# liuQuan98/APR

Hardware: AMD Instinct MI355X
Metric: point-cloud pairs/sec (120k-pt KITTI frame, FCGF encode+match+SVD) (higher is better)
Workload: dtype f32

## Files before the change

apr_amd/_lib.py:

```python
from __future__ import annotations

import ctypes as C
import os

import torch

_HERE = os.path.dirname(os.path.abspath(__file__))
LIB_PATH = os.path.join(_HERE, "lib", "libapr_hip.so")

_p = C.c_void_p
_i32, _i64, _u64, _f32, _f64, _sz = C.c_int32, C.c_int64, C.c_uint64, C.c_float, C.c_double, C.c_size_t

class PairDesc(C.Structure):
    _fields_ = [("f0", C.c_void_p), ("n0", C.c_int64), ("f1", C.c_void_p), ("n1", C.c_int64),
                ("xyz0", C.c_void_p), ("xyz1", C.c_void_p), ("seed", C.c_uint64)]


class SpconvDesc(C.Structure):
    _fields_ = [("inp", C.c_void_p), ("ldi", C.c_int64), ("nbr", C.c_void_p), ("n_out", C.c_int64),
                ("K", C.c_int32), ("cin", C.c_int32), ("cout", C.c_int32), ("relu", C.c_int32),
                ("w_packed", C.c_void_p), ("scale", C.c_void_p), ("shift", C.c_void_p),
                ("residual", C.c_void_p), ("ldr", C.c_int64), ("out", C.c_void_p), ("ldo", C.c_int64),
                ("counters", C.c_void_p), ("plist", C.c_void_p), ("prod_scratch", C.c_void_p),
                ("plist_bytes", C.c_int64), ("w_bf3", C.c_void_p),
# ... 21 lines not shown
    _fields_ = [("layer", ResunetLayer * 23), ("conv1_w", C.c_void_p), ("conv1_ks", C.c_int32), ("normalize", C.c_int32),
                ("ws_conv", C.c_uint32), ("ws_block", C.c_uint32), ("os_block", C.c_uint32),
                ("ws3", C.c_int32), ("ws3_cin128", C.c_int32), ("os_min_rows", C.c_int32), ("occ_kernel_map", C.c_int32),
                ("ws3_max_rows_128", C.c_int64)]


class LevelMap(C.Structure):
    _fields_ = [("coords", C.c_void_p), ("keys", C.c_void_p), ("vals", C.c_void_p), ("cap", C.c_int64), ("n", C.c_int64)]


class Pyramid(C.Structure):
    _fields_ = [("lv", LevelMap * 4), ("first", C.c_void_p), ("pts", C.c_void_p), ("header", C.c_void_p),
                ("header_ints", C.c_int32), ("compact", C.c_int32), ("compact_rows", C.c_int64),
                ("counters", C.c_void_p), ("n_counter_slots", C.c_int32)]


class GcnLayer(C.Structure):
    _fields_ = [("kind", C.c_int32), ("k", C.c_int32), ("heads", C.c_int32),
                ("eps1", C.c_float), ("eps2", C.c_float), ("eps3", C.c_float),
                ("w1", C.c_void_p), ("w2", C.c_void_p), ("w3", C.c_void_p), ("b1", C.c_void_p), ("b2", C.c_void_p),
                ("wq", C.c_void_p), ("wk", C.c_void_p), ("wv", C.c_void_p), ("wm", C.c_void_p),
                ("bq", C.c_void_p), ("bk", C.c_void_p), ("bv", C.c_void_p), ("bm", C.c_void_p)]


class GcnDesc(C.Structure):
    _fields_ = [("n_layers", C.c_int32), ("c", C.c_int32), ("layer", GcnLayer * 8)]


PROTOTYPES = {
    "apr_col_sums": (C.c_int, [_p, _i64, _i64, _i32, _p, _p, _sz, _p]),
    "apr_mha_train_forward": (C.c_int, [_p, _p, _p, _i32, _i32, _i32, _i32, _i32, _p, _p, _p]),
    "apr_mha_train_backward": (C.c_int, [_p, _p, _p, _p, _p, _i32, _i32, _i32, _i32, _i32, _p, _p, _p, _p, _p]),
    "apr_edge_features_backward": (C.c_int, [_p, _i32, _i32, _i32, _p, _i64, _p, _p]),
    "apr_gcn_scratch_bytes": (_sz, [_p, _i32, _i32]),
    "apr_gcn_forward": (C.c_int, [_p, _p, _i32, _p, _i32, _p, _i64, _p, _i64, _p, _i64, _p, _i64, _p, _sz, _p]),
    "apr_voxel_pyramid_scratch_bytes": (_sz, [_i64, _i32]),
    "apr_voxel_pyramid": (C.c_int, [_p, _p, _i32, _f32, _p, _sz, _p, _p]),
    "apr_resunet_encode_supported": (C.c_int, [_p, _p, _p]),
    "apr_resunet_encode_scratch_bytes": (_sz, [_p, _p, _p]),
    "apr_resunet_encode": (C.c_int, [_p, _p, _p, _p, _i32, _p, _sz, _p, _i64, _p]),
    "apr_last_error": (C.c_char_p, []),
    "apr_version": (C.c_int, []),
    "apr_device_count": (C.c_int, []),
    "apr_struct_sizes": (_i32, [_p, _i32]),
    "apr_ransac_set_screen": (C.c_int, [_i32]),
    "apr_ransac_set_option": (C.c_int, [_i32, _i32]),
    "apr_ransac_sampling_launches": (C.c_int, [_p]),
    "apr_event_wait": (C.c_int, [_p, _i32]),
    "apr_event_wait_timeout": (C.c_int, [_p, _i32, _i64]),
    "apr_hash_capacity": (_i64, [_i64]),
    "apr_map_scratch_bytes": (_sz, [_i64]),
    "apr_voxelize": (C.c_int, [_p, _i64, _f32, _i32, _p, _p]),
    "apr_map_build": (C.c_int, [_p, _i64, _p, _i32, _p, _p, _i64, _p, _p, _p, _p, _p, _sz, _p]),
    "apr_kernel_map_transpose": (C.c_int, [_p, _i64, _i32, _i64, _p, _p]),
    "apr_voxelize_segments": (C.c_int, [_p, _i64, C.c_float, _p, _i32, _p, _p]),
    "apr_segment_counts": (C.c_int, [_p, _p, _p, _i32, _p, _p]),
    "apr_kernel_map_same": (C.c_int, [_p, _i64, _p, _p, _i64, _i32, _i32, _p, _p]),
    "apr_kernel_map": (C.c_int, [_p, _i64, _p, _p, _p, _i64, _i32, _i32, _p, _p]),
    "apr_spconv_packed_size": (_i64, [_i32, _i32, _i32]),
    "apr_spconv_pack_weights": (C.c_int, [_p, _i32, _i32, _i32, _p, _p]),
    "apr_spconv_fwd": (C.c_int, [_p, _i64, _p, _i64, _i32, _i32, _i32, _p, _p, _p, _p, _i64, _i32, _p, _i64, _p]),
    "apr_pairlist_counter_ints": (_i32, []),
    "apr_pairlist_bytes": (_sz, [_i64, _i32]),
    "apr_pairlist_build": (C.c_int, [_p, _i64, _i32, _p, _p, _sz, _p]),
    "apr_pairlist3_bytes": (_sz, [_i64]),
    "apr_pairlist3_build": (C.c_int, [_p, _i64, _i32, _p, _p, _sz, _p]),
    "apr_spconv_ws3_supported": (C.c_int, [_i32, _i32, _i32]),
    "apr_spconv_ws3_fwd_bf3": (C.c_int, [_p, _i64, _p, _p, _i64, _i32, _i32, _p, _p, _p, _p, _i64, _i32, _p, _i64, _p, _p]),
    "apr_spconv_ws_fwd": (C.c_int, [_p, _i64, _p, _p, _i64, _i32, _i32, _i32, _p, _p, _p, _p, _i64, _i32, _p, _i64, _p, _p]),
    "apr_spconv_packed_bf3_bytes": (_i64, [_i32, _i32, _i32]),
    "apr_spconv_pack_weights_bf3": (C.c_int, [_p, _i32, _i32, _i32, _p, _p]),
    "apr_spconv_pack_weights_bf3_ex": (C.c_int, [_p, _i32, _i32, _i32, _i32, _i32, _p, _p]),
    "apr_spconv_ws_fwd_bf3": (C.c_int, [_p, _i64, _p, _p, _i64, _i32, _i32, _i32, _p, _p, _p, _p, _p, _i64, _i32, _p, _i64,
                                        _p, _p]),
    "apr_spconv_wgrad_scratch_bytes": (_sz, [_i64, _i32, _i32, _i32]),
    "apr_spconv_wgrad": (C.c_int, [_p, _i64, _p, _i64, _p, _i64, _i32, _i32, _i32, _p, _p, _sz, _p]),
    "apr_spconv_wgrad_same_level": (C.c_int, [_p, _i64, _p, _i64, _p, _i64, _i32, _i32, _i32, _p, _p, _sz, _p]),
    "apr_spconv_route": (_i32, [_p]),
    "apr_spconv_tile_variant": (_i32, [_p]),
    "apr_dense_gemm_bf3_variant": (_i32, [_i64, _i32, _i32]),
    "apr_spconv_wgrad_plan": (C.c_int, [_p, _i64, _p, _i64, _i64, _i32, _i32, _i32, _i32, _p]),
    "apr_spconv_ws_supported": (_i32, [_i32, _i32, _i32]),
    "apr_spconv_bigk_supported": (_i32, [_i32, _i32, _i32]),
    "apr_spconv_fwd_batch": (C.c_int, [_p, _i32, _p]),
    "apr_spconv_fwd_batch_timed": (C.c_int, [_p, _i32, _p, _p]),
    "apr_bn_stats": (C.c_int, [_p, _i64, _i64, _i32, _p, _p, _p, _sz, _p]),
    "apr_norm_params": (C.c_int, [_p, _i64, _i64, _i32, _f32, _p, _p, _p, _sz, _p]),
    "apr_bn_stats_scratch_bytes": (_sz, [_i64, _i32]),
    "apr_instance_norm_act": (C.c_int, [_p, _i64, _i64, _i32, _f32, _p, _i64, _i32, _f32, _p, _i64, _p, _sz, _p]),
    "apr_spconv_os_tile_rows": (_i32, [_i64, _i32, _i32]),
    "apr_spconv_os_pairs_bytes": (_sz, [_i64, _i32, _i32]),
    "apr_spconv_os_pairs_build": (C.c_int, [_p, _i64, _i64, _i32, _i32, _p, _sz, _p]),
    "apr_spconv_os_trace": (C.c_int, [_p, _i32]),
    "apr_spconv_os_set_debug": (C.c_int, [_i32]),
    "apr_spconv_os_fwd": (C.c_int, [_p, _i64, _p, _i64, _i32, _i32, _i32, _i32, _p, _p, _p, _p, _i64, _i32, _p, _i64, _p]),
    "apr_norm_backward_scratch_bytes": (_sz, [_i64, _i32]),
    "apr_norm_backward": (C.c_int, [_p, _i64, _p, _i64, _i64, _i32, _p, _p, _p, _p, _i64, _p, _p, _p, _sz, _p]),
    "apr_bn_train_fwd": (C.c_int, [_p, _i64, _i64, _i32, _p, _p, C.c_float, C.c_float, _p, _p, _p, _i64, _i32, _p, _i64, _p, _p,
                                   _p, _p, _i32, _p, _sz, _p]),
    "apr_bn_train_bwd": (C.c_int, [_p, _i64, _p, _i64, _p, _i64, _i64, _i32, _p, _p, _p, _i32, _p, _i64, _p, _i64, _p, _p,
                                   _p, _i32, _p, _sz, _p]),
    "apr_weights_flip_transpose": (C.c_int, [_p, _i32, _i32, _i32, _i32, _p, _p]),
    "apr_dense_gemm_bf3": (C.c_int, [_p, _i64, _i64, _i32, _i32, _p, _p, _p, _p, _i64, _i32, _p, _i64, _p]),
    "apr_dense_rows_bf3_ok": (_i32, [_i32, _i32]),
    "apr_dense_rows_bf3_route": (_i32, [_i64, _i32, _i32]),
    "apr_dense_rows_bf3": (C.c_int, [_p, _i64, _i64, _i32, _i32, _p, _p, _p, _p, _i64, _i32, _i32, _p, _i64, _p]),
# ... 195 lines not shown
```

apr_amd/csrc/encoder.hip:

```cpp
#include "common.h"

namespace {

constexpr int kLevels = 4, kStages = 7, kMaps = 10, kMaxLists = 24;

struct ListSlot {
  int map, kind, rows;
  void* blob;
  size_t bytes;
  int32_t* counters;
  bool built;
};

struct Enc {
  const apr_resunet_plan& P;
  const apr_level_map* lv;
  const int32_t* bbox;
  AprArena arena;
  const bool dry;
  hipStream_t st;
  int rc = APR_OK;

  int32_t* kmap[kMaps] = {};
  ListSlot lists[kMaxLists];
  int nlists = 0, ncounter = 0;
  int32_t* counters = nullptr;
  int n_counter_slots = 0;
  void* occ = nullptr;
  size_t occ_bytes = 0;
  int32_t* tpool[3] = {};
  bool tpool_ready = false;
  float* prod = nullptr;
  size_t prod_bytes = 0;

  apr_spconv_desc descs[4];
  int ndesc = 0;

  Enc(const apr_resunet_plan& p, const apr_level_map* l, const int32_t* b, void* scratch, hipStream_t s)
      : P(p), lv(l), bbox(b), arena(scratch), dry(scratch == nullptr), st(s) {}

  float* rows(int64_t n, int c) { return arena.take<float>((size_t)n * c); }
  size_t need() const { return arena.bytes() + apr_align256(prod_bytes); }
  bool ok() const { return rc == APR_OK; }
  void run(int r) {
    if (rc == APR_OK && r != APR_OK) rc = r;
  }

  int64_t map_rows(int m) const { return m < 4 ? lv[m].n : m < 7 ? lv[m - 4 + 1].n : lv[m - 7].n; }
  int64_t map_in_rows(int m) const { return m < 4 ? lv[m].n : m < 7 ? lv[m - 4].n : lv[m - 7 + 1].n; }

  int32_t* kernel_map(int m) {
    if (kmap[m] || (dry && kmap_sized[m])) return kmap[m];
    kmap_sized[m] = true;
    const int64_t n_out = map_rows(m);
    if (m >= 7) {
      const int l = m - 7;
      int32_t* fwd = kernel_map(4 + l);
      if (!tpool_ready) {
        size_t ints = 0;
        for (int a = 0; a < 3; ++a) ints += (size_t)lv[a].n * 27;
        ints = (ints + 63) / 64 * 64 + 64;
        int32_t* buf = arena.take<int32_t>(ints);
        size_t pos = 0;
        for (int a = 0; a < 3; ++a) {
          tpool[a] = dry ? nullptr : buf + pos;
          pos += (size_t)lv[a].n * 27;
        }
        if (!dry) run(apr_fill_bytes(buf, 0xFF, ints * 4, st));
        tpool_ready = true;
      }
      kmap[m] = tpool[l];
      if (!dry) run(apr_kernel_map_transpose_prefilled(fwd, lv[l + 1].n, 27, lv[l].n, kmap[m], st));
      return kmap[m];
    }
    kmap[m] = arena.take<int32_t>((size_t)n_out * 27);
    if (dry) return kmap[m];
    const int lin = m < 4 ? m : m - 4, lout = m < 4 ? m : m - 4 + 1;
    const apr_level_map& in = lv[lin];
    const apr_level_map& outm = lv[lout];
    if (lin == 0 && P.occ_kernel_map && occ)
      run(apr_kernel_map_occ(outm.coords, outm.n, nullptr, in.keys, in.vals, in.cap, 3, 1, bbox, P.conv1_ks, occ, kmap[m], st));
    else
      run(apr_kernel_map(outm.coords, outm.n, nullptr, in.keys, in.vals, in.cap, 3, 1 << lin, kmap[m], st));
    return kmap[m];
  }
  bool kmap_sized[kMaps] = {};

  ListSlot* find_list(int m, int kind, int rws) {
    for (int i = 0; i < nlists; ++i)
      if (lists[i].map == m && lists[i].kind == kind && lists[i].rows == rws) return &lists[i];
    return nullptr;
  }

  ListSlot* ws_list(const apr_resunet_layer& L, int m, bool same_level) {
    bool tri = P.ws3 && L.w_bf3 && apr_spconv_ws3_supported(L.K, L.cin, L.cout);
    if (tri && L.cin == 128 && ((same_level && map_rows(m) > P.ws3_max_rows_128) || !P.ws3_cin128)) tri = false;
    const int kind = tri ? 1 : 0;
    ListSlot* s = find_list(m, kind, 0);
    if (s) return s;
    if (nlists >= kMaxLists) {
      apr_set_error("apr_resunet_encode: more than %d pair lists", kMaxLists);
      run(APR_EINVAL);
      return nullptr;
    }
    s = &lists[nlists++];
    s->map = m;
    s->kind = kind;
    s->rows = 0;
    s->bytes = tri ? apr_pairlist3_bytes(map_rows(m)) : apr_pairlist_bytes(map_rows(m), 27);
    s->blob = arena.take<char>(s->bytes);
    s->built = false;
    s->counters = nullptr;
    if (!dry) {
      if (ncounter >= n_counter_slots) {
        apr_set_error("apr_resunet_encode: more than %d pair lists need a counter block", n_counter_slots);
        run(APR_EINVAL);
        return nullptr;
      }
      s->counters = counters + (size_t)ncounter * apr_pairlist_counter_ints();
    }
    ++ncounter;
    return s;
  }

  ListSlot* os_list(const apr_resunet_layer& L, int m) {
    const int64_t n_out = map_rows(m), n_in = map_in_rows(m);
    const int rws = n_in < (1ll << 23) ? apr_spconv_os_tile_rows(n_out, L.cin, L.cout) : 0;
    if (rws <= 0) return nullptr;
    ListSlot* s = find_list(m, 2, rws);
    if (s) return s;
    if (nlists >= kMaxLists) {
      apr_set_error("apr_resunet_encode: more than %d pair lists", kMaxLists);
      run(APR_EINVAL);
      return nullptr;
    }
    s = &lists[nlists++];
// ... 130 lines not shown
  const apr_resunet_layer* L = p->layer;
  for (int s = 0; s < kStages; ++s)
    if (L[3 * s + 1].cin != L[3 * s].cout || L[3 * s + 1].cout != L[3 * s].cout || L[3 * s + 2].cin != L[3 * s].cout ||
        L[3 * s + 2].cout != L[3 * s].cout)
      return false;
  if (L[3].cin != L[0].cout || L[6].cin != L[3].cout || L[9].cin != L[6].cout || L[12].cin != L[9].cout ||
      L[15].cin != L[12].cout + L[6].cout || L[18].cin != L[15].cout + L[3].cout || L[21].cin != L[18].cout + L[0].cout ||
      L[22].cin != L[21].cout)
    return false;
  if (L[0].cin != 1 || L[0].K != p->conv1_ks * p->conv1_ks * p->conv1_ks || L[0].cout % 8 != 0) return false;
  if (p->conv1_ks != 3 && p->conv1_ks != 5 && p->conv1_ks != 7) return false;
  return true;
}

}

APR_API int apr_resunet_encode_supported(const apr_resunet_plan* plan, const apr_level_map* lv, const int32_t* bbox_host) {
  if (!plan_ok(plan, lv, bbox_host)) return 0;
  return apr_occ_conv_pays(bbox_host, plan->conv1_ks, lv[0].n) ? 1 : 0;
}

APR_API size_t apr_resunet_encode_scratch_bytes(const apr_resunet_plan* plan, const apr_level_map* lv, const int32_t* bbox_host) {
  if (!apr_resunet_encode_supported(plan, lv, bbox_host)) return 0;
  Enc e(*plan, lv, bbox_host, nullptr, nullptr);
  e.walk(nullptr, plan->layer[22].cout);
  return e.need();
}

APR_API int apr_resunet_encode(const apr_resunet_plan* plan, const apr_level_map* lv, const int32_t* bbox_host, int32_t* counters,
                               int32_t n_counter_slots, void* scratch, size_t scratch_bytes, float* out, int64_t ldo,
                               void* stream) {
  APR_CHECK_ARG(apr_resunet_encode_supported(plan, lv, bbox_host),
                "apr_resunet_encode: plan / maps / box not covered (apr_resunet_encode_supported)");
  APR_CHECK_ARG(scratch && out && ldo >= plan->layer[22].cout && (!counters || n_counter_slots > 0),
                "apr_resunet_encode: bad arguments");
  Enc dry(*plan, lv, bbox_host, nullptr, nullptr);
  dry.walk(nullptr, ldo);
  APR_CHECK_ARG(scratch_bytes >= dry.need(), "apr_resunet_encode: scratch too small");
  Enc e(*plan, lv, bbox_host, scratch, (hipStream_t)stream);
  e.counters = counters;
  e.n_counter_slots = counters ? n_counter_slots : 0;
  e.prod_bytes_live = dry.prod_bytes;
  e.walk(out, ldo);
  return e.rc;
}

namespace {

struct MapBufs {
  uint64_t* keys; int32_t* vals; int64_t cap; int32_t* coords; int64_t* first; int32_t *n_dev, *status; void* scratch;
  size_t scratch_bytes; int64_t rows;
};

MapBufs take_map(AprArena& f, int64_t rows, bool want_first, int32_t* hdr_slot, void* shared_scratch, size_t shared_bytes) {
  MapBufs m;
  m.rows = rows;
  m.cap = apr_hash_capacity(rows);
  m.keys = f.take<uint64_t>((size_t)m.cap);
  m.vals = f.take<int32_t>((size_t)m.cap);
  m.coords = f.take<int32_t>((size_t)rows * 4);
  m.first = want_first ? f.take<int64_t>((size_t)rows) : nullptr;
  m.scratch_bytes = shared_bytes;
  m.scratch = shared_scratch;
  m.n_dev = hdr_slot;
  m.status = hdr_slot ? hdr_slot + 1 : nullptr;
  return m;
}

inline int64_t compact_rows_for(int64_t n_points) { return n_points > 4 * 65536 ? (n_points / 4 > 65536 ? n_points / 4 : 65536) : 0; }

int front_walk(AprArena& f, const float* const* frames, const int64_t* offs, int32_t nseg, float vs, apr_pyramid* out,
               hipStream_t st) {
  const int64_t N = offs ? offs[nseg] : 0;
  const int64_t R = compact_rows_for(N);
  const int hints = 10 + nseg + 8;
  const bool dry = f.base == nullptr;
  int32_t* hdr = f.take<int32_t>((size_t)hints);
  int32_t* counters = f.take<int32_t>((size_t)16 * apr_pairlist_counter_ints());
  int32_t* raw = f.take<int32_t>((size_t)N * 4);
  int64_t* offs_dev = f.take<int64_t>((size_t)(nseg + 1));
  float* pts = f.take<float>((size_t)N * 3);
  const size_t sbytes = apr_map_scratch_bytes(N);
  void* const sc = f.take<char>(sbytes);
  MapBufs dedup = take_map(f, N, true, dry ? nullptr : hdr + (R ? 8 : 0), sc, sbytes);
  MapBufs lvl[4];
  if (R) lvl[0] = take_map(f, R, false, dry ? nullptr : hdr, sc, sbytes);
  else lvl[0] = dedup;
  const int64_t rows = R ? R : N;
  for (int l = 1; l < 4; ++l) lvl[l] = take_map(f, rows, false, dry ? nullptr : hdr + 2 * l, sc, sbytes);
  if (dry) return APR_OK;

  int rc;
  const size_t clear = (size_t)((char*)counters - (char*)hdr) + (size_t)16 * apr_pairlist_counter_ints() * 4;
  if ((rc = apr_pack_i32(nullptr, nullptr, 0, nullptr, hdr, (int64_t)(clear / 4), st)) != APR_OK) return rc;
  if ((rc = apr_voxelize_frames(frames, offs, nseg, vs, raw, offs_dev, st)) != APR_OK) return rc;
  if ((rc = apr_map_build(raw, N, nullptr, 0, dedup.keys, dedup.vals, dedup.cap, dedup.coords, dedup.first, dedup.n_dev,
                          dedup.status, dedup.scratch, dedup.scratch_bytes, st)) != APR_OK)
    return rc;
  if ((rc = apr_segment_counts(dedup.first, dedup.n_dev, offs_dev, nseg, hdr + 10, st)) != APR_OK) return rc;
  if ((rc = apr_coords_bbox(raw, N, hdr + 10 + nseg, st)) != APR_OK) return rc;
  if ((rc = apr_gather_frame_points(frames, offs, nseg, dedup.first, dedup.n_dev, N, pts, st)) != APR_OK) return rc;
  if (R &&
      (rc = apr_map_build(dedup.coords, R, dedup.n_dev, 0, lvl[0].keys, lvl[0].vals, lvl[0].cap, lvl[0].coords, nullptr,
                          lvl[0].n_dev, lvl[0].status, lvl[0].scratch, lvl[0].scratch_bytes, st)) != APR_OK)
    return rc;
  for (int l = 1; l < 4; ++l)
    if ((rc = apr_map_build(lvl[l - 1].coords, rows, lvl[l - 1].n_dev, 1 << l, lvl[l].keys, lvl[l].vals, lvl[l].cap, lvl[l].coords,
                            nullptr, lvl[l].n_dev, lvl[l].status, lvl[l].scratch, lvl[l].scratch_bytes, st)) != APR_OK)
      return rc;
  for (int l = 0; l < 4; ++l) {
    out->lv[l].coords = lvl[l].coords; out->lv[l].keys = lvl[l].keys; out->lv[l].vals = lvl[l].vals;
    out->lv[l].cap = lvl[l].cap; out->lv[l].n = lvl[l].rows;
  }
  out->first = dedup.first;
  out->pts = pts;
  out->header = hdr;
  out->header_ints = hints;
  out->compact = R ? 1 : 0;
  out->compact_rows = R;
  out->counters = counters;
  out->n_counter_slots = 16;
  return APR_OK;
}

}

APR_API size_t apr_voxel_pyramid_scratch_bytes(int64_t n_points, int32_t nseg) {
  if (n_points <= 0 || nseg <= 0 || nseg > APR_MAX_FRAMES) return 0;
  AprArena f(nullptr);
  int64_t offs[APR_MAX_FRAMES + 1] = {};
  offs[nseg] = n_points;
  (void)front_walk(f, nullptr, offs, nseg, 1.f, nullptr, nullptr);
  return f.bytes();
}

APR_API int apr_voxel_pyramid(const float* const* frames_host, const int64_t* offsets_host, int32_t nseg, float voxel_size,
                              void* arena, size_t arena_bytes, apr_pyramid* out, void* stream) {
  APR_CHECK_ARG(frames_host && offsets_host && nseg >= 1 && nseg <= APR_MAX_FRAMES && arena && out && voxel_size > 0.f,
                "apr_voxel_pyramid: bad arguments (1 .. %d frames)", APR_MAX_FRAMES);
  APR_CHECK_ARG(offsets_host[0] == 0 && offsets_host[nseg] > 0, "apr_voxel_pyramid: offsets must run 0 .. total points > 0");
  APR_CHECK_ARG(arena_bytes >= apr_voxel_pyramid_scratch_bytes(offsets_host[nseg], nseg), "apr_voxel_pyramid: arena too small");
  AprArena f(arena);
  return front_walk(f, frames_host, offsets_host, nseg, voxel_size, out, (hipStream_t)stream);
}
```

apr_amd/csrc/hash.hip:

```cpp
#include "common.h"

namespace {

constexpr int kBlock = 256;

__global__ void k_voxelize(const float* __restrict__ xyz, int64_t n, float vs, int batch,
                           int4* __restrict__ coords) {
  int64_t i = (int64_t)blockIdx.x * blockDim.x + threadIdx.x;
  if (i >= n) return;
  float x = xyz[3 * i + 0] / vs, y = xyz[3 * i + 1] / vs, z = xyz[3 * i + 2] / vs;
  coords[i] = make_int4(batch, (int)floorf(x), (int)floorf(y), (int)floorf(z));
}

__global__ void k_voxelize_segments(const float* __restrict__ xyz, int64_t n, float vs,
                                    const long long* __restrict__ offsets, int nseg, int4* __restrict__ coords) {
  int64_t i = (int64_t)blockIdx.x * blockDim.x + threadIdx.x;
  if (i >= n) return;
  int b = 0;
  while (b + 1 < nseg && i >= offsets[b + 1]) ++b;
  float x = xyz[3 * i + 0] / vs, y = xyz[3 * i + 1] / vs, z = xyz[3 * i + 2] / vs;
  coords[i] = make_int4(b, (int)floorf(x), (int)floorf(y), (int)floorf(z));
}

__device__ inline int4 load_coord(const int4* coords, int64_t i, int floor_to) {
// ... 173 lines not shown
  int64_t total = n_out * K;
  if (n_out_dev) total = (int64_t)min((long long)n_out, (long long)*n_out_dev) * K;
  for (int64_t t = (int64_t)blockIdx.x * blockDim.x + threadIdx.x; t < total;
       t += (int64_t)gridDim.x * blockDim.x) {
    int64_t j = t / K;
    int o = (int)(t - j * K);
    int ox = o % ks - h, oy = (o / ks) % ks - h, oz = o / (ks * ks) - h;
    int4 c = out_coords[j];
    int x = c.y + ox * scale, y = c.z + oy * scale, z = c.w + oz * scale;
    int r = -1;
    if (apr_key_in_range(c.x, x, y, z)) r = table_lookup(keys, vals, mask, apr_pack_key(c.x, x, y, z));
    nbr[t] = r;
  }
}

__global__ void k_kernel_map_sym(const int4* __restrict__ coords, int64_t n, const unsigned long long* __restrict__ keys,
                                 const int* __restrict__ vals, uint32_t mask, int ks, int scale,
                                 int* __restrict__ nbr) {
  const int K = ks * ks * ks, h = ks / 2, half = K / 2;
  const int64_t total = n * (half + 1);
  for (int64_t t = (int64_t)blockIdx.x * blockDim.x + threadIdx.x; t < total;
       t += (int64_t)gridDim.x * blockDim.x) {
    const int64_t j = t / (half + 1);
    const int o = (int)(t - j * (half + 1));
    if (o == half) {
      nbr[j * K + o] = (int)j;
      continue;
    }
    const int ox = o % ks - h, oy = (o / ks) % ks - h, oz = o / (ks * ks) - h;
    const int4 c = coords[j];
    const int x = c.y + ox * scale, y = c.z + oy * scale, z = c.w + oz * scale;
    int r = -1;
    if (apr_key_in_range(c.x, x, y, z)) r = table_lookup(keys, vals, mask, apr_pack_key(c.x, x, y, z));
    nbr[j * K + o] = r;
    if (r >= 0) nbr[(int64_t)r * K + (K - 1 - o)] = (int)j;
  }
}

__global__ void k_fill_upper(int* __restrict__ nbr, int64_t n, int K, int half) {
  const int64_t total = n * half;
  for (int64_t t = (int64_t)blockIdx.x * blockDim.x + threadIdx.x; t < total; t += (int64_t)gridDim.x * blockDim.x) {
    const int64_t j = t / half;
    nbr[j * K + half + 1 + (int)(t - j * half)] = -1;
  }
}

__global__ void k_map_transpose(const int* __restrict__ nbr, int64_t total, int K, int* __restrict__ nbr_t) {
  const int64_t t = (int64_t)blockIdx.x * blockDim.x + threadIdx.x;
  if (t >= total) return;
  const int i = nbr[t];
  if (i >= 0) nbr_t[(int64_t)i * K + (int)(t % K)] = (int)(t / K);
}

constexpr int kMaxFrames = APR_MAX_FRAMES;
struct FrameTable {
  const float* ptr[kMaxFrames];
  long long off[kMaxFrames + 1];
  int nseg;
};

__device__ inline int frame_of(const FrameTable& ft, long long i) {
  int b = 0;
  while (b + 1 < ft.nseg && i >= ft.off[b + 1]) ++b;
  return b;
}

__global__ void k_voxelize_frames(FrameTable ft, int64_t n, float vs, int4* __restrict__ coords,
                                  long long* __restrict__ offsets_out) {
  int64_t i = (int64_t)blockIdx.x * blockDim.x + threadIdx.x;
  if (blockIdx.x == 0 && threadIdx.x <= ft.nseg && offsets_out) offsets_out[threadIdx.x] = ft.off[threadIdx.x];
  if (i >= n) return;
  const int b = frame_of(ft, i);
  const float* p = ft.ptr[b] + 3 * (i - ft.off[b]);
  float x = p[0] / vs, y = p[1] / vs, z = p[2] / vs;
  coords[i] = make_int4(b, (int)floorf(x), (int)floorf(y), (int)floorf(z));
}

__global__ void k_gather_frame_points(FrameTable ft, const long long* __restrict__ first, const int* __restrict__ n_dev,
                                      float* __restrict__ pts) {
  const int64_t r = (int64_t)blockIdx.x * blockDim.x + threadIdx.x;
  if (r >= *n_dev) return;
  const long long i = first[r];
  const int b = frame_of(ft, i);
  const float* p = ft.ptr[b] + 3 * (i - ft.off[b]);
  pts[3 * r + 0] = p[0];
  pts[3 * r + 1] = p[1];
  pts[3 * r + 2] = p[2];
}

constexpr int kMaxPack = APR_MAX_PACK;
struct PackTable {
  const int* src[kMaxPack];
  int begin[kMaxPack + 1];
  int nsrc;
};
__global__ void k_pack_i32(PackTable pt, int* __restrict__ dst, int* __restrict__ zero_ptr, long long zero_words) {
  for (int s = 0; s < pt.nsrc; ++s) {
    const int n = pt.begin[s + 1] - pt.begin[s];
    for (int e = blockIdx.x * blockDim.x + threadIdx.x; e < n; e += gridDim.x * blockDim.x) dst[pt.begin[s] + e] = pt.src[s][e];
  }
  for (long long e = (long long)blockIdx.x * blockDim.x + threadIdx.x; e < zero_words; e += (long long)gridDim.x * blockDim.x)
    zero_ptr[e] = 0;
}

}

// ... 18 lines not shown
  m.blk_off = a.take<int>(nblk);
  return m;
}
}

APR_API size_t apr_map_scratch_bytes(int64_t n) {
  AprArena a(nullptr);
  walk_map(a, n);
  return a.bytes();
}

APR_API int apr_voxelize(const float* xyz, int64_t n, float voxel_size, int32_t batch,
                         int32_t* coords, void* stream) {
  APR_CHECK_ARG(n >= 0 && voxel_size > 0.f, "apr_voxelize: bad n=%lld or voxel_size", (long long)n);
  APR_CHECK_ARG(batch >= 0 && batch < 1023, "apr_voxelize: batch index %d outside [0,1023)", batch);
  if (n == 0) return APR_OK;
  hipLaunchKernelGGL(k_voxelize, dim3((unsigned)cdiv64(n, kBlock)), dim3(kBlock), 0, (hipStream_t)stream,
                     xyz, n, voxel_size, batch, (int4*)coords);
  APR_LAUNCH_CHECK();
  return APR_OK;
}

APR_API int apr_map_build(const int32_t* coords_in, int64_t n, const int32_t* n_dev, int32_t floor_to,
                          uint64_t* keys,
                          int32_t* vals, int64_t cap, int32_t* out_coords, int64_t* out_first,
                          int32_t* n_out, int32_t* status, void* scratch, size_t scratch_bytes,
                          void* stream) {
  hipStream_t st = (hipStream_t)stream;
  APR_CHECK_ARG(n >= 0 && n < (1ll << 31), "apr_map_build: n=%lld out of range", (long long)n);
  APR_CHECK_ARG(cap >= 2 * n && (cap & (cap - 1)) == 0, "apr_map_build: cap=%lld must be a power of two >= 2n",
                (long long)cap);
  AprArena arena(scratch);
  const MapScratch m = walk_map(arena, n);
  APR_CHECK_ARG(arena.fits(scratch_bytes), "apr_map_build: scratch too small");
  APR_CHECK_ARG(floor_to >= 0, "apr_map_build: floor_to < 0");
  hipLaunchKernelGGL(k_table_init, dim3((unsigned)cdiv64(cap, 256)), dim3(256), 0, st, (unsigned long long*)keys, vals,
                     cap, status, n == 0 ? n_out : (int*)nullptr);
  if (n == 0) {
    APR_LAUNCH_CHECK();
    return APR_OK;
  }
  const int nblk = (int)cdiv64(n, kBlock);
  const uint32_t mask = (uint32_t)(cap - 1);
  hipLaunchKernelGGL(k_insert, dim3(nblk), dim3(kBlock), 0, st, (const int4*)coords_in, n, n_dev,
                     floor_to, (unsigned long long*)keys, vals, mask, m.slot_of, status);
  hipLaunchKernelGGL(k_flag_count, dim3(nblk), dim3(kBlock), 0, st, vals, m.slot_of, n, n_dev, m.flags, m.blk_cnt);
  hipLaunchKernelGGL(k_scan_blocks, dim3(1), dim3(1024), 0, st, m.blk_cnt, nblk, m.blk_off, n_out);
  hipLaunchKernelGGL(k_compact, dim3(nblk), dim3(kBlock), 0, st, (const int4*)coords_in, n, n_dev, floor_to,
                     m.flags, m.blk_off, m.slot_of, vals, (int4*)out_coords, (long long*)out_first);
  APR_LAUNCH_CHECK();
  return APR_OK;
}

static int map_transpose(const int32_t* nbr, int64_t n_out, int32_t K, int64_t n_in, int32_t* nbr_t, bool prefilled,
                         void* stream) {
  APR_CHECK_ARG(n_out >= 0 && n_in >= 0 && K >= 1 && (nbr || n_out == 0) && (nbr_t || n_in == 0),
                "apr_kernel_map_transpose: bad arguments");
  hipStream_t st = (hipStream_t)stream;
  if (n_in > 0 && !prefilled) {
    if (int rcf = apr_internal_fill(nbr_t, 0xFF, (size_t)n_in * K * 4, st)) return rcf;
  }
  if (n_out > 0)
    hipLaunchKernelGGL(k_map_transpose, dim3((unsigned)cdiv64(n_out * K, kBlock)), dim3(kBlock), 0, st, nbr,
                       n_out * (int64_t)K, K, nbr_t);
  APR_LAUNCH_CHECK();
  return APR_OK;
}

APR_API int apr_kernel_map_transpose(const int32_t* nbr, int64_t n_out, int32_t K, int64_t n_in, int32_t* nbr_t,
                                     void* stream) {
  return map_transpose(nbr, n_out, K, n_in, nbr_t, false, stream);
}

APR_API int apr_kernel_map_transpose_prefilled(const int32_t* nbr, int64_t n_out, int32_t K, int64_t n_in, int32_t* nbr_t,
                                               void* stream) {
  return map_transpose(nbr, n_out, K, n_in, nbr_t, true, stream);
}

static __global__ __launch_bounds__(256) void k_fill_bytes(unsigned char* __restrict__ p, unsigned v32, unsigned long long head,
                                              unsigned long long n16, unsigned long long tail) {
  uint4* const q = (uint4*)(p + head);
  const uint4 v = make_uint4(v32, v32, v32, v32);
  for (unsigned long long i = (unsigned long long)blockIdx.x * blockDim.x + threadIdx.x; i < n16;
       i += (unsigned long long)gridDim.x * blockDim.x)
    q[i] = v;
  if (blockIdx.x == 0) {
    if (threadIdx.x < head) p[threadIdx.x] = (unsigned char)v32;
    if (threadIdx.x < tail) p[head + n16 * 16 + threadIdx.x] = (unsigned char)v32;
  }
}

int apr_internal_fill(void* ptr, int32_t byte_value, size_t bytes, hipStream_t st) {
  static const int s_kernel = env_int("APR_FILL_KERNEL", 1);
  if (bytes == 0) return APR_OK;
  if (!s_kernel) {
    APR_HIP(hipMemsetAsync(ptr, byte_value, bytes, st));
    return APR_OK;
  }
  const unsigned b = (unsigned)byte_value & 0xFFu;
  const unsigned v32 = b * 0x01010101u;
  size_t head = (16 - ((uintptr_t)ptr & 15)) & 15;
  if (head > bytes) head = bytes;
  const size_t n16 = (bytes - head) / 16, tail = bytes - head - n16 * 16;
  int64_t nblk = cdiv64((int64_t)n16, 256 * 8);
  nblk = nblk < 1 ? 1 : (nblk > 2048 ? 2048 : nblk);
  hipLaunchKernelGGL(k_fill_bytes, dim3((unsigned)nblk), dim3(256), 0, st, (unsigned char*)ptr, v32, (unsigned long long)head,
// ... 131 lines not shown
```

include/apr_hip.h:

```cpp
#ifndef APR_HIP_H
#define APR_HIP_H

#include <stddef.h>
#include <stdint.h>

#ifdef __cplusplus
extern "C" {
#endif

#define APR_OK 0
#define APR_EINVAL (-1)
#define APR_EHIP (-2)
#define APR_ETIMEOUT (-3)
#define APR_ERANGE (-3)

const char* apr_last_error(void);
int apr_version(void);
int apr_device_count(void);
int32_t apr_struct_sizes(int32_t* out, int32_t n);
int apr_event_wait(void* event, int32_t poll_us);
int apr_event_wait_timeout(void* event, int32_t poll_us, int64_t timeout_us);


int64_t apr_hash_capacity(int64_t n);

size_t apr_map_scratch_bytes(int64_t n);

int apr_voxelize(const float* xyz, int64_t n, float voxel_size, int32_t batch,
                 int32_t* coords, void* stream);

int apr_map_build(const int32_t* coords_in, int64_t n, const int32_t* n_dev, int32_t floor_to,
                  uint64_t* keys, int32_t* vals, int64_t cap,
                  int32_t* out_coords, int64_t* out_first, int32_t* n_out,
                  int32_t* status, void* scratch, size_t scratch_bytes, void* stream);

int apr_kernel_map_transpose(const int32_t* nbr, int64_t n_out, int32_t K, int64_t n_in, int32_t* nbr_t, void* stream);

int apr_voxelize_segments(const float* xyz, int64_t n, float voxel_size, const int64_t* offsets, int32_t nseg,
                          int32_t* coords, void* stream);

#define APR_MAX_FRAMES 64
int apr_voxelize_frames(const float* const* frames_host, const int64_t* offsets_host, int32_t nseg, float voxel_size,
                        int32_t* coords, int64_t* offsets_dev, void* stream);
int apr_gather_frame_points(const float* const* frames_host, const int64_t* offsets_host, int32_t nseg,
                            const int64_t* out_first, const int32_t* n_dev, int64_t n_max, float* pts, void* stream);

#define APR_MAX_PACK 96
int apr_pack_i32(const int32_t* const* srcs_host, const int32_t* counts_host, int32_t nsrc, int32_t* dst,
                 int32_t* zero_ptr, int64_t zero_words, void* stream);
int apr_fill_bytes(void* ptr, int32_t byte_value, size_t bytes, void* stream);
int apr_kernel_map_transpose_prefilled(const int32_t* nbr, int64_t n_out, int32_t K, int64_t n_in, int32_t* nbr_t,
                                       void* stream);

int apr_segment_counts(const int64_t* out_first, const int32_t* n_dev, const int64_t* offsets, int32_t nseg,
                       int32_t* counts, void* stream);

int apr_kernel_map_same(const int32_t* coords, int64_t n, const uint64_t* keys, const int32_t* vals, int64_t cap,
                        int32_t kernel_size, int32_t scale, int32_t* nbr, void* stream);
int apr_kernel_map(const int32_t* out_coords, int64_t n_out, const int32_t* n_out_dev,
                   const uint64_t* in_keys, const int32_t* in_vals, int64_t cap,
                   int32_t kernel_size, int32_t scale, int32_t* nbr, void* stream);

int apr_coords_bbox(const int32_t* coords, int64_t n, int32_t* bbox_dev, void* stream);
size_t apr_occ_conv_scratch_bytes(const int32_t* bbox_host, int32_t kernel_size);
int apr_occ_conv_pays(const int32_t* bbox_host, int32_t kernel_size, int64_t n);
int apr_occ_conv(const int32_t* coords, int64_t n, const int32_t* bbox_host, int32_t kernel_size, const float* w,
                 int32_t cout, const float* scale, const float* shift, const float* residual, int64_t ldr,
                 int32_t relu, float* out, int64_t ldo, void* scratch, size_t scratch_bytes, void* stream);
int apr_kernel_map_occ(const int32_t* out_coords, int64_t n_out, const int32_t* n_out_dev, const uint64_t* in_keys,
                       const int32_t* in_vals, int64_t cap, int32_t kernel_size, int32_t scale,
                       const int32_t* bbox_host, int32_t bitmap_kernel_size, const void* occ_scratch, int32_t* nbr,
                       void* stream);


int64_t apr_spconv_packed_size(int32_t K, int32_t cin, int32_t cout);
int apr_spconv_pack_weights(const float* w, int32_t K, int32_t cin, int32_t cout,
                            float* w_packed, void* stream);

int apr_weights_flip_transpose(const float* w, int32_t K, int32_t cin, int32_t cout, int32_t flip, float* wt, void* stream);

int apr_spconv_fwd(const float* in, int64_t ldi, const int32_t* nbr, int64_t n_out,
                   int32_t K, int32_t cin, int32_t cout, const float* w_packed,
                   const float* scale, const float* shift,
                   const float* residual, int64_t ldr, int32_t relu,
                   float* out, int64_t ldo, void* stream);

#define APR_PAIR_COUNTER_STRIDE 64
int32_t apr_pairlist_counter_ints(void);
size_t apr_pairlist_bytes(int64_t n_out, int32_t K);
int apr_pairlist_build(const int32_t* nbr, int64_t n_out, int32_t K, int32_t* counters, void* plist,
                       size_t plist_bytes, void* stream);
int apr_spconv_ws_fwd(const float* in, int64_t ldi, const int32_t* counters, const void* plist, int64_t n_out,
                      int32_t K, int32_t cin,
                      int32_t cout, const float* w_packed, const float* scale, const float* shift,
                      const float* residual, int64_t ldr, int32_t relu, float* out, int64_t ldo,
                      float* prod_scratch, void* stream);
int64_t apr_spconv_packed_bf3_bytes(int32_t K, int32_t cin, int32_t cout);
int apr_spconv_pack_weights_bf3(const float* w, int32_t K, int32_t cin, int32_t cout, void* w_bf3, void* stream);
int apr_spconv_pack_weights_bf3_ex(const float* w, int32_t K, int32_t cin, int32_t cout, int32_t flip, int32_t transposed,
                                   void* w_bf3, void* stream);
int apr_spconv_ws_fwd_bf3(const float* in, int64_t ldi, const int32_t* counters, const void* plist, int64_t n_out,
                          int32_t K, int32_t cin, int32_t cout, const float* w_packed, const void* w_bf3,
                          const float* scale, const float* shift, const float* residual, int64_t ldr, int32_t relu,
                          float* out, int64_t ldo, float* prod_scratch, void* stream);

int32_t apr_spconv_os_tile_rows(int64_t n_out, int32_t cin, int32_t cout);
size_t apr_spconv_os_pairs_bytes(int64_t n_out, int32_t K, int32_t R);
int apr_spconv_os_pairs_build(const int32_t* nbr, int64_t n_out, int64_t n_in, int32_t K, int32_t R, void* os_pairs,
                              size_t os_pairs_bytes, void* stream);
int apr_spconv_os_trace(uint64_t* host_out, int32_t n);
int apr_spconv_os_set_debug(int32_t mode);
int apr_spconv_os_fwd(const float* in, int64_t ldi, const void* os_pairs, int64_t n_out, int32_t K, int32_t R,
                      int32_t cin, int32_t cout, const void* w_bf3, const float* scale, const float* shift,
                      const float* residual, int64_t ldr, int32_t relu, float* out, int64_t ldo, void* stream);
// ... 529 lines not shown
```

Measured before the change: 2674.

## Build strided-down and transposed kernel maps in one fine-to-coarse pass

```diff
diff --git a/apr_amd/_lib.py b/apr_amd/_lib.py
--- a/apr_amd/_lib.py
+++ b/apr_amd/_lib.py
@@ -97,6 +97,8 @@
     "apr_map_scratch_bytes": (_sz, [_i64]),
     "apr_voxelize": (C.c_int, [_p, _i64, _f32, _i32, _p, _p]),
     "apr_map_build": (C.c_int, [_p, _i64, _p, _i32, _p, _p, _i64, _p, _p, _p, _p, _p, _sz, _p]),
+    "apr_map_insert_unique": (C.c_int, [_p, _i64, _p, _p, _p, _i64, _p, _p, _p]),
+    "apr_kernel_map_down": (C.c_int, [_p, _i64, _p, _p, _i64, _i64, _i32, _p, _p, _p]),
     "apr_kernel_map_transpose": (C.c_int, [_p, _i64, _i32, _i64, _p, _p]),
     "apr_voxelize_segments": (C.c_int, [_p, _i64, C.c_float, _p, _i32, _p, _p]),
     "apr_segment_counts": (C.c_int, [_p, _p, _p, _i32, _p, _p]),
diff --git a/apr_amd/csrc/encoder.hip b/apr_amd/csrc/encoder.hip
--- a/apr_amd/csrc/encoder.hip
+++ b/apr_amd/csrc/encoder.hip
@@ -28,8 +28,8 @@
   int n_counter_slots = 0;
   void* occ = nullptr;
   size_t occ_bytes = 0;
-  int32_t* tpool[3] = {};
-  bool tpool_ready = false;
+  int32_t* dpool[6] = {};
+  bool dpool_ready = false;
   float* prod = nullptr;
   size_t prod_bytes = 0;
 
@@ -53,35 +53,41 @@
     if (kmap[m] || (dry && kmap_sized[m])) return kmap[m];
     kmap_sized[m] = true;
     const int64_t n_out = map_rows(m);
-    if (m >= 7) {
-      const int l = m - 7;
-      int32_t* fwd = kernel_map(4 + l);
-      if (!tpool_ready) {
+    if (m >= 4) {
+      const int l = (m - 4) % 3;
+      if (!dpool_ready) {
         size_t ints = 0;
+        for (int a = 0; a < 3; ++a) ints += ((size_t)lv[a + 1].n * 27 + 63) / 64 * 64;
         for (int a = 0; a < 3; ++a) ints += (size_t)lv[a].n * 27;
         ints = (ints + 63) / 64 * 64 + 64;
         int32_t* buf = arena.take<int32_t>(ints);
         size_t pos = 0;
         for (int a = 0; a < 3; ++a) {
-          tpool[a] = dry ? nullptr : buf + pos;
+          dpool[a] = dry ? nullptr : buf + pos;
+          pos += ((size_t)lv[a + 1].n * 27 + 63) / 64 * 64;
+        }
+        for (int a = 0; a < 3; ++a) {
+          dpool[3 + a] = dry ? nullptr : buf + pos;
           pos += (size_t)lv[a].n * 27;
         }
         if (!dry) run(apr_fill_bytes(buf, 0xFF, ints * 4, st));
-        tpool_ready = true;
+        dpool_ready = true;
       }
-      kmap[m] = tpool[l];
-      if (!dry) run(apr_kernel_map_transpose_prefilled(fwd, lv[l + 1].n, 27, lv[l].n, kmap[m], st));
+      kmap[4 + l] = dpool[l];
+      kmap[7 + l] = dpool[3 + l];
+      kmap_sized[4 + l] = kmap_sized[7 + l] = true;
+      if (!dry)
+        run(apr_kernel_map_down(lv[l].coords, lv[l].n, lv[l + 1].keys, lv[l + 1].vals, lv[l + 1].cap, lv[l + 1].n, 1 << l,
+                                kmap[4 + l], kmap[7 + l], st));
       return kmap[m];
     }
     kmap[m] = arena.take<int32_t>((size_t)n_out * 27);
     if (dry) return kmap[m];
-    const int lin = m < 4 ? m : m - 4, lout = m < 4 ? m : m - 4 + 1;
-    const apr_level_map& in = lv[lin];
-    const apr_level_map& outm = lv[lout];
-    if (lin == 0 && P.occ_kernel_map && occ)
-      run(apr_kernel_map_occ(outm.coords, outm.n, nullptr, in.keys, in.vals, in.cap, 3, 1, bbox, P.conv1_ks, occ, kmap[m], st));
+    const apr_level_map& in = lv[m];
+    if (m == 0 && P.occ_kernel_map && occ)
+      run(apr_kernel_map_occ(in.coords, in.n, nullptr, in.keys, in.vals, in.cap, 3, 1, bbox, P.conv1_ks, occ, kmap[m], st));
     else
-      run(apr_kernel_map(outm.coords, outm.n, nullptr, in.keys, in.vals, in.cap, 3, 1 << lin, kmap[m], st));
+      run(apr_kernel_map(in.coords, in.n, nullptr, in.keys, in.vals, in.cap, 3, 1 << m, kmap[m], st));
     return kmap[m];
   }
   bool kmap_sized[kMaps] = {};
@@ -318,13 +324,14 @@
   size_t scratch_bytes; int64_t rows;
 };
 
-MapBufs take_map(AprArena& f, int64_t rows, bool want_first, int32_t* hdr_slot, void* shared_scratch, size_t shared_bytes) {
+MapBufs take_map(AprArena& f, int64_t rows, bool want_first, int32_t* hdr_slot, void* shared_scratch, size_t shared_bytes,
+                 bool alias = false, int32_t* alias_coords = nullptr) {
   MapBufs m;
   m.rows = rows;
   m.cap = apr_hash_capacity(rows);
   m.keys = f.take<uint64_t>((size_t)m.cap);
   m.vals = f.take<int32_t>((size_t)m.cap);
-  m.coords = f.take<int32_t>((size_t)rows * 4);
+  m.coords = alias ? alias_coords : f.take<int32_t>((size_t)rows * 4);
   m.first = want_first ? f.take<int64_t>((size_t)rows) : nullptr;
   m.scratch_bytes = shared_bytes;
   m.scratch = shared_scratch;
@@ -350,7 +357,7 @@
   void* const sc = f.take<char>(sbytes);
   MapBufs dedup = take_map(f, N, true, dry ? nullptr : hdr + (R ? 8 : 0), sc, sbytes);
   MapBufs lvl[4];
-  if (R) lvl[0] = take_map(f, R, false, dry ? nullptr : hdr, sc, sbytes);
+  if (R) lvl[0] = take_map(f, R, false, dry ? nullptr : hdr, sc, sbytes, true, dedup.coords);
   else lvl[0] = dedup;
   const int64_t rows = R ? R : N;
   for (int l = 1; l < 4; ++l) lvl[l] = take_map(f, rows, false, dry ? nullptr : hdr + 2 * l, sc, sbytes);
@@ -366,9 +373,8 @@
   if ((rc = apr_segment_counts(dedup.first, dedup.n_dev, offs_dev, nseg, hdr + 10, st)) != APR_OK) return rc;
   if ((rc = apr_coords_bbox(raw, N, hdr + 10 + nseg, st)) != APR_OK) return rc;
   if ((rc = apr_gather_frame_points(frames, offs, nseg, dedup.first, dedup.n_dev, N, pts, st)) != APR_OK) return rc;
-  if (R &&
-      (rc = apr_map_build(dedup.coords, R, dedup.n_dev, 0, lvl[0].keys, lvl[0].vals, lvl[0].cap, lvl[0].coords, nullptr,
-                          lvl[0].n_dev, lvl[0].status, lvl[0].scratch, lvl[0].scratch_bytes, st)) != APR_OK)
+  if (R && (rc = apr_map_insert_unique(dedup.coords, R, dedup.n_dev, lvl[0].keys, lvl[0].vals, lvl[0].cap, lvl[0].n_dev,
+                                       lvl[0].status, st)) != APR_OK)
     return rc;
   for (int l = 1; l < 4; ++l)
     if ((rc = apr_map_build(lvl[l - 1].coords, rows, lvl[l - 1].n_dev, 1 << l, lvl[l].keys, lvl[l].vals, lvl[l].cap, lvl[l].coords,
diff --git a/apr_amd/csrc/hash.hip b/apr_amd/csrc/hash.hip
--- a/apr_amd/csrc/hash.hip
+++ b/apr_amd/csrc/hash.hip
@@ -249,6 +249,56 @@
   if (i >= 0) nbr_t[(int64_t)i * K + (int)(t % K)] = (int)(t / K);
 }
 
+__global__ void k_insert_unique(const int4* __restrict__ coords, int64_t n, const int* __restrict__ n_dev,
+                                unsigned long long* __restrict__ keys, int* __restrict__ vals, uint32_t mask,
+                                int* __restrict__ n_out, int* __restrict__ status) {
+  const int64_t i = (int64_t)blockIdx.x * blockDim.x + threadIdx.x;
+  if (n_dev) n = min((long long)n, (long long)max(*n_dev, 0));
+  if (i == 0) *n_out = (int)n;
+  if (i >= n) return;
+  const int4 c = coords[i];
+  if (!apr_key_in_range(c.x, c.y, c.z, c.w)) {
+    *status = 1;
+    return;
+  }
+  const unsigned long long key = apr_pack_key(c.x, c.y, c.z, c.w);
+  uint32_t sl = apr_hash_u64(key) & mask;
+  for (uint32_t probe = 0; probe <= mask; ++probe) {
+    if (keys[sl] == APR_KEY_EMPTY && atomicCAS(&keys[sl], APR_KEY_EMPTY, key) == APR_KEY_EMPTY) {
+      vals[sl] = (int)i;
+      return;
+    }
+    sl = (sl + 1) & mask;
+  }
+  *status = 2;
+}
+
+__global__ void k_kernel_map_down(const int4* __restrict__ fine, int64_t n_f, int64_t n_c,
+                                  const unsigned long long* __restrict__ keys, const int* __restrict__ vals, uint32_t mask,
+                                  int s, int* __restrict__ nbr, int* __restrict__ nbr_t) {
+  const int64_t total = n_f * 8;
+  const int s2 = 2 * s;
+  for (int64_t t = (int64_t)blockIdx.x * blockDim.x + threadIdx.x; t < total; t += (int64_t)gridDim.x * blockDim.x) {
+    const int64_t i = t >> 3;
+    const int cand = (int)(t & 7);
+    const int4 f = fine[i];
+    if (!apr_key_in_range(f.x, f.y, f.z, f.w)) continue;
+    const int cx = apr_floor_to(f.y, s2), cy = apr_floor_to(f.z, s2), cz = apr_floor_to(f.w, s2);
+    const int rx = f.y - cx, ry = f.z - cy, rz = f.w - cz;
+    if ((rx != 0 && rx != s) || (ry != 0 && ry != s) || (rz != 0 && rz != s)) continue;
+    const int bx = cand & 1, by = (cand >> 1) & 1, bz = cand >> 2;
+    if ((bx && rx == 0) || (by && ry == 0) || (bz && rz == 0)) continue;
+    const int X = cx + bx * s2, Y = cy + by * s2, Z = cz + bz * s2;
+    if (!apr_key_in_range(f.x, X, Y, Z)) continue;
+    const int j = table_lookup(keys, vals, mask, apr_pack_key(f.x, X, Y, Z));
+    if (j < 0 || j >= n_c) continue;
+    const int ox = rx == 0 ? 0 : (bx ? -1 : 1), oy = ry == 0 ? 0 : (by ? -1 : 1), oz = rz == 0 ? 0 : (bz ? -1 : 1);
+    const int k = (ox + 1) + 3 * (oy + 1) + 9 * (oz + 1);
+    nbr[(int64_t)j * 27 + k] = (int)i;
+    nbr_t[i * 27 + k] = j;
+  }
+}
+
 constexpr int kMaxFrames = APR_MAX_FRAMES;
 struct FrameTable {
   const float* ptr[kMaxFrames];
@@ -373,6 +423,37 @@
   return APR_OK;
 }
 
+APR_API int apr_map_insert_unique(const int32_t* coords, int64_t n, const int32_t* n_dev, uint64_t* keys, int32_t* vals,
+                                  int64_t cap, int32_t* n_out, int32_t* status, void* stream) {
+  hipStream_t st = (hipStream_t)stream;
+  APR_CHECK_ARG(n >= 0 && n < (1ll << 31) && n_out && status && keys && vals && (coords || n == 0),
+                "apr_map_insert_unique: bad arguments (n=%lld)", (long long)n);
+  APR_CHECK_ARG(cap >= 2 * n && cap > 0 && (cap & (cap - 1)) == 0 && cap <= (1ll << 31),
+                "apr_map_insert_unique: cap=%lld must be a power of two >= 2n", (long long)cap);
+  hipLaunchKernelGGL(k_table_init, dim3((unsigned)cdiv64(cap, 256)), dim3(256), 0, st, (unsigned long long*)keys, vals,
+                     cap, status, n_out);
+  if (n > 0)
+    hipLaunchKernelGGL(k_insert_unique, dim3((unsigned)cdiv64(n, kBlock)), dim3(kBlock), 0, st, (const int4*)coords, n, n_dev,
+                       (unsigned long long*)keys, vals, (uint32_t)(cap - 1), n_out, status);
+  APR_LAUNCH_CHECK();
+  return APR_OK;
+}
+
+APR_API int apr_kernel_map_down(const int32_t* fine_coords, int64_t n_f, const uint64_t* coarse_keys, const int32_t* coarse_vals,
+                                int64_t cap, int64_t n_c, int32_t stride, int32_t* nbr, int32_t* nbr_t, void* stream) {
+  APR_CHECK_ARG(n_f >= 0 && n_f < (1ll << 31) && n_c >= 0 && n_c < (1ll << 31), "apr_kernel_map_down: bad row counts");
+  APR_CHECK_ARG((cap & (cap - 1)) == 0 && cap > 0 && cap <= (1ll << 31), "apr_kernel_map_down: cap must be a power of two");
+  APR_CHECK_ARG(stride >= 1 && stride <= (1 << 15), "apr_kernel_map_down: stride=%d outside [1, 2^15]", stride);
+  if (n_f == 0 || n_c == 0) return APR_OK;
+  APR_CHECK_ARG(fine_coords && coarse_keys && coarse_vals && nbr && nbr_t, "apr_kernel_map_down: null pointer");
+  int64_t nblk = cdiv64(n_f * 8, kBlock);
+  if (nblk > 65536) nblk = 65536;
+  hipLaunchKernelGGL(k_kernel_map_down, dim3((unsigned)nblk), dim3(kBlock), 0, (hipStream_t)stream, (const int4*)fine_coords,
+                     n_f, n_c, (const unsigned long long*)coarse_keys, coarse_vals, (uint32_t)(cap - 1), stride, nbr, nbr_t);
+  APR_LAUNCH_CHECK();
+  return APR_OK;
+}
+
 static int map_transpose(const int32_t* nbr, int64_t n_out, int32_t K, int64_t n_in, int32_t* nbr_t, bool prefilled,
                          void* stream) {
   APR_CHECK_ARG(n_out >= 0 && n_in >= 0 && K >= 1 && (nbr || n_out == 0) && (nbr_t || n_in == 0),
diff --git a/include/apr_hip.h b/include/apr_hip.h
--- a/include/apr_hip.h
+++ b/include/apr_hip.h
@@ -34,6 +34,9 @@
                   int32_t* out_coords, int64_t* out_first, int32_t* n_out,
                   int32_t* status, void* scratch, size_t scratch_bytes, void* stream);
 
+int apr_map_insert_unique(const int32_t* coords, int64_t n, const int32_t* n_dev, uint64_t* keys, int32_t* vals,
+                          int64_t cap, int32_t* n_out, int32_t* status, void* stream);
+
 int apr_kernel_map_transpose(const int32_t* nbr, int64_t n_out, int32_t K, int64_t n_in, int32_t* nbr_t, void* stream);
 
 int apr_voxelize_segments(const float* xyz, int64_t n, float voxel_size, const int64_t* offsets, int32_t nseg,
@@ -60,6 +63,9 @@
 int apr_kernel_map(const int32_t* out_coords, int64_t n_out, const int32_t* n_out_dev,
                    const uint64_t* in_keys, const int32_t* in_vals, int64_t cap,
                    int32_t kernel_size, int32_t scale, int32_t* nbr, void* stream);
+
+int apr_kernel_map_down(const int32_t* fine_coords, int64_t n_f, const uint64_t* coarse_keys, const int32_t* coarse_vals,
+                        int64_t cap, int64_t n_c, int32_t stride, int32_t* nbr, int32_t* nbr_t, void* stream);
 
 int apr_coords_bbox(const int32_t* coords, int64_t n, int32_t* bbox_dev, void* stream);
 size_t apr_occ_conv_scratch_bytes(const int32_t* bbox_host, int32_t kernel_size);
```

After: 2663. About the same (-0.4%).
